# ma-compbio/MATCHA

Hardware: AMD Instinct MI355X
Metric: training hyperedges/sec at k∈{2..5}, embed_dim=64; 1/2/4/8 MI355X (higher is better)
Workload: dtype f32; 1 GPU; hg38_1mb bins (N=3067), k in {2,3,4,5} mixed-k zero-padded to L=5, embed_dim=64, front end=table, neg_num=3, dropout on, AdamW lr=1e-3, 400000 known hyperedges; parallelism=dp1, hipgraph=False, table_gradient_exchange=none, embedding_backward=float atomics, exchange_overlapped=False

## Files before the change

matcha_amd/csrc/tail_bwd.hip:

```cpp
#include "bf16x3.hpp"
#include "kernels.hpp"
#include "loss_reduce.hpp"

namespace matcha {

namespace {

constexpr int kLd = 68;
constexpr int kTileF = 32 * kLd;
constexpr int kPS = 80;
constexpr int kPlane = 32 * kPS;
constexpr int kPT = 3 * kPlane;
constexpr float kEps = 1e-5f;
constexpr int kSlab = 2 * 4096 + 10 * 64;
constexpr int kVec = 2 * 4096;
typedef Planes<kPS, 16> PL;

struct TailBwdArgs {
  const float* dH2; const float* Y; const float* H1;
  const int32_t* count; const int32_t* half_meta; const int32_t* tok_slot;
  int nhalves;
  const float* W0; const float* W1;
  const uint64_t* seed; float p_fc1, p_pff;
  float* ddyn0; float* slab;
  float* zero_rows;
  int64_t zero_floats;
  const float* row_loss; int64_t B; float* losses; int zero_recon;
  const float* vslab;
};
constexpr size_t kLdsBytes = (size_t)2 * kTileF * 4 + (size_t)4 * kPT * 2;

__global__ __launch_bounds__(256) __attribute__((amdgpu_waves_per_eu(2, 2))) void tail_bwd64_kernel(TailBwdArgs g) {
  extern __shared__ __attribute__((aligned(16))) float lds[];
  float* Hs = lds;
  float* Ds = lds + kTileF;
  short* Dp = reinterpret_cast<short*>(lds + 2 * kTileF);
  short* Hp = Dp + kPT;
  short* Yp = Hp + kPT;
  short* Zp = Yp + kPT;

  const int tid = threadIdx.x;
  const int nwg = (int)gridDim.x - (g.losses ? 1 : 0);
  if ((int)blockIdx.x == nwg) {
    loss_reduce_role<256>(g.row_loss, g.B, g.losses, g.zero_recon, lds);
    return;
  }
  const int tr = g.count[1];
  int nh = g.count[3];
  if (nh > g.nhalves) nh = g.nhalves;
  const int per = (nh + nwg - 1) / nwg;
  const int tile_lo = blockIdx.x * per;
  const int tile_hi = tile_lo + per < nh ? tile_lo + per : nh;

  if (g.zero_floats > 0) {
    f32x4* z = reinterpret_cast<f32x4*>(g.zero_rows);
    const int64_t n4 = g.zero_floats >> 2;
    for (int64_t i = (int64_t)blockIdx.x * 256 + tid; i < n4; i += (int64_t)nwg * 256) z[i] = (f32x4){0.f, 0.f, 0.f, 0.f};
  }
  const bool zero_tok = g.zero_rows && g.zero_floats == 0;
  if (blockIdx.x == 0 && tid < 16)
    *reinterpret_cast<f32x4*>(g.ddyn0 + (int64_t)tr * 64 + 4 * tid) = (f32x4){0.f, 0.f, 0.f, 0.f};
  const bool drop1 = g.p_fc1 > 0.f, drop2 = g.p_pff > 0.f;
  uint32_t key1 = 0, key2 = 0, thr1 = 0, thr2 = 0;
  float ks1 = 1.f, ks2 = 1.f;
  if (drop1 || drop2) {
    const uint64_t seed = *g.seed;
    key1 = rng_key(seed, kStreamDropFc1); key2 = rng_key(seed, kStreamDropPff);
    if (drop1) { thr1 = dropout_threshold(g.p_fc1); ks1 = 1.f / (1.f - g.p_fc1); }
    if (drop2) { thr2 = dropout_threshold(g.p_pff); ks2 = 1.f / (1.f - g.p_pff); }
  }
  const float unscale = drop2 ? 1.f - g.p_pff : 1.f;

  f32x4 aw1[4], aw0[4];
#pragma unroll
  for (int i = 0; i < 4; ++i) { aw1[i] = (f32x4){0.f, 0.f, 0.f, 0.f}; aw0[i] = aw1[i]; }
  float va0 = 0.f, va1 = 0.f, va2 = 0.f;
  V8 a_c1 = zero8();
  f32x4 a_c0 = {0.f, 0.f, 0.f, 0.f};

  Frag3 W1f[2], W0f[2];
  {
    const int lane = tid & 63, wave = tid >> 6, c16 = lane & 15, kq = lane >> 4, fb = 16 * wave;
    const float* p1 = g.W1 + (8 * kq) * 64 + fb + c16;
    const float* p0 = g.W0 + (8 * kq) * 64 + fb + c16;
#pragma unroll
    for (int s = 0; s < 2; ++s) {
      float v1[8], v0[8];
#pragma unroll
      for (int j = 0; j < 8; ++j) { v1[j] = p1[(32 * s + j) * 64]; v0[j] = p0[(32 * s + j) * 64]; }
      W1f[s] = split8(v1); W0f[s] = split8(v0);
    }
  }

  const int4* meta = reinterpret_cast<const int4*>(g.half_meta);
  const int4 mzero = make_int4(0, 0, 0, 0);
  int4 mc = tile_lo < tile_hi ? meta[tile_lo] : mzero;
  int4 mn = tile_lo + 1 < tile_hi ? meta[tile_lo + 1] : mzero;
  V8 yn, hn, dn;
  uint32_t sn0 = 0, sn1 = 0;
#define TB_GLOAD(M)                                                                                      \
  do {                                                                                                   \
    const int row__ = tid >> 3, sub__ = tid & 7;                                                         \
    const int64_t tok__ = (M).x + (row__ < (M).y ? row__ : ((M).y > 0 ? (M).y - 1 : 0));                  \
    const int64_t o__ = tok__ * 64 + 8 * sub__;                                                          \
    yn = ld8(g.Y + o__); hn = ld8(g.H1 + o__); dn = ld8(g.dH2 + o__);                                    \
    if (drop1 || drop2) {      \
      const int c16__ = tid & 15;                                                                        \
      sn0 = (uint32_t)g.tok_slot[(M).x + (c16__ < (M).y ? c16__ : 0)];                                   \
      sn1 = (uint32_t)g.tok_slot[(M).x + (16 + c16__ < (M).y ? 16 + c16__ : 0)];                         \
    }                                                                                                    \
  } while (0)
  TB_GLOAD(mc);
  V8 yq = yn, hq = hn, dq = dn;
  uint32_t sq0 = sn0, sq1 = sn1;
  {
    const V8 ty = yn, th = hn, td = dn; const uint32_t t0_ = sn0, t1_ = sn1;
    TB_GLOAD(mn);
    yq = yn; hq = hn; dq = dn; sq0 = sn0; sq1 = sn1;
    yn = ty; hn = th; dn = td; sn0 = t0_; sn1 = t1_;
  }

  for (int tile = tile_lo; tile < tile_hi; ++tile) {
    const int4 mnn = tile + 2 < tile_hi ? meta[tile + 2] : mzero;
    const int t0 = mc.x, n_real = mc.y;
    const float* vs = g.vslab + (int64_t)tile * kSlab + kVec;
    const float vl0 = vs[tid], vl1 = vs[tid + 256], vl2 = tid == 64 ? vs[9 * 64] : 0.f;
    int tid_ = tid;
    asm volatile("" : "+v"(tid_));
    const int lane = tid_ & 63, wave = tid_ >> 6;
    const int c16 = lane & 15, kq = lane >> 4, fb = 16 * wave;
    const int row = tid_ >> 3, sub = tid_ & 7;
    {
      const V8 dh2 = scale8(row < n_real ? 1.f : 0.f, dn);
      if (zero_tok && row < n_real) st8(g.zero_rows + ((int64_t)t0 + row) * 64 + 8 * sub, zero8());
      add8(a_c1, dh2);
      st8(&Ds[row * kLd + 8 * sub], dh2);
      st8(&Hs[row * kLd + 8 * sub], hn);
      PL::store(Dp + row * kPS + 8 * sub, split8(dh2));
      PL::store(Hp + row * kPS + 8 * sub, split8(hn));
      PL::store(Yp + row * kPS + 8 * sub, split8(yn));
    }
    const uint32_t slot0 = sn0, slot1 = sn1;
    __syncthreads();
    yn = yq; hn = hq; dn = dq; sn0 = sq0; sn1 = sq1;
    {
      const V8 ty = yn, th = hn, td = dn; const uint32_t t0_ = sn0, t1_ = sn1;
      TB_GLOAD(mnn);
      yq = yn; hq = hn; dq = dn; sq0 = sn0; sq1 = sn1;
      yn = ty; hn = th; dn = td; sn0 = t0_; sn1 = t1_;
    }
    {
      f32x4 acc0 = {0.f, 0.f, 0.f, 0.f}, acc1 = acc0;
      const short* dp = Dp + c16 * kPS + 8 * kq;
#pragma unroll
      for (int s = 0; s < 2; ++s) {
        const Frag3 b0 = PL::row(dp + 32 * s), b1 = PL::row(dp + 16 * kPS + 32 * s);
        acc0 = mma6(acc0, W1f[s], b0); acc1 = mma6(acc1, W1f[s], b1);
      }
      const f32x4 hv0 = *reinterpret_cast<const f32x4*>(&Hs[c16 * kLd + fb + 4 * kq]);
      const f32x4 hv1 = *reinterpret_cast<const f32x4*>(&Hs[(16 + c16) * kLd + fb + 4 * kq]);
      const uint32_t hr0 = lowbias32(slot0 ^ key2), hr1 = lowbias32(slot1 ^ key2);
#pragma unroll
      for (int e = 0; e < 4; ++e) {
        const uint32_t f = (uint32_t)(fb + 4 * kq + e);
        float v0 = acc0[e], v1 = acc1[e];
        if (drop2) {
          v0 = lowbias32(f ^ hr0) >= thr2 ? v0 * ks2 : 0.f;
          v1 = lowbias32(f ^ hr1) >= thr2 ? v1 * ks2 : 0.f;
        }
        const float t0_ = hv0[e] * unscale, t1_ = hv1[e] * unscale;
        acc0[e] = v0 * (1.f - t0_ * t0_); acc1[e] = v1 * (1.f - t1_ * t1_);
      }
      a_c0 += acc0 + acc1;
      {
        const P3 p0 = split2(acc0[0], acc0[1]), p1 = split2(acc0[2], acc0[3]);
        short* d = Zp + c16 * kPS + fb + 4 * kq;
        *reinterpret_cast<u32x2*>(d) = (u32x2){p0.h, p1.h}; *reinterpret_cast<u32x2*>(d + kPlane) = (u32x2){p0.m, p1.m};
        *reinterpret_cast<u32x2*>(d + 2 * kPlane) = (u32x2){p0.l, p1.l};
      }
      {
        const P3 p0 = split2(acc1[0], acc1[1]), p1 = split2(acc1[2], acc1[3]);
        short* d = Zp + (16 + c16) * kPS + fb + 4 * kq;
        *reinterpret_cast<u32x2*>(d) = (u32x2){p0.h, p1.h}; *reinterpret_cast<u32x2*>(d + kPlane) = (u32x2){p0.m, p1.m};
        *reinterpret_cast<u32x2*>(d + 2 * kPlane) = (u32x2){p0.l, p1.l};
      }
    }
    __syncthreads();
    {
      f32x4 acc0 = *reinterpret_cast<const f32x4*>(&Ds[c16 * kLd + fb + 4 * kq]);
      f32x4 acc1 = *reinterpret_cast<const f32x4*>(&Ds[(16 + c16) * kLd + fb + 4 * kq]);
      const short* zp = Zp + c16 * kPS + 8 * kq;
#pragma unroll
      for (int s = 0; s < 2; ++s) {
        const Frag3 b0 = PL::row(zp + 32 * s), b1 = PL::row(zp + 16 * kPS + 32 * s);
        acc0 = mma6(acc0, W0f[s], b0); acc1 = mma6(acc1, W0f[s], b1);
      }
      if (drop1) {
        const uint32_t hr0 = lowbias32(slot0 ^ key1), hr1 = lowbias32(slot1 ^ key1);
#pragma unroll
        for (int e = 0; e < 4; ++e) {
          const uint32_t f = (uint32_t)(fb + 4 * kq + e);
          acc0[e] = lowbias32(f ^ hr0) >= thr1 ? acc0[e] * ks1 : 0.f;
          acc1[e] = lowbias32(f ^ hr1) >= thr1 ? acc1[e] * ks1 : 0.f;
        }
      }
      float* out = g.ddyn0 + ((int64_t)t0 + c16) * 64 + fb + 4 * kq;
      if (c16 < n_real) *reinterpret_cast<f32x4*>(out) = acc0;
      if (16 + c16 < n_real) *reinterpret_cast<f32x4*>(out + 16 * 64) = acc1;
    }
    {
      const int blk = ((4 * kq + ((lane & 15) >> 2)) * kPS) + 4 * (lane & 3);
      const Frag3 hb = PL::col(Hp + blk + fb), yb = PL::col(Yp + blk + fb);
#pragma unroll
      for (int i = 0; i < 4; ++i) aw1[i] = mma6(aw1[i], PL::col(Dp + blk + 16 * i), hb);
#pragma unroll
      for (int i = 0; i < 4; ++i) aw0[i] = mma6(aw0[i], PL::col(Zp + blk + 16 * i), yb);
    }
    __syncthreads();
    va0 += vl0; va1 += vl1; va2 += vl2;
    mc = mn; mn = mnn;
  }
#undef TB_GLOAD

  const int lane = tid & 63, wave = tid >> 6, c16 = lane & 15, kq = lane >> 4, fb = 16 * wave;
  float* slab = g.slab + (int64_t)blockIdx.x * kSlab;
  {
    const int col = fb + c16;
#pragma unroll
    for (int i = 0; i < 4; ++i)
#pragma unroll
      for (int reg = 0; reg < 4; ++reg) {
        const int rw = 16 * i + 4 * kq + reg;
        slab[rw * 64 + col] = aw1[i][reg];
        slab[4096 + rw * 64 + col] = aw0[i][reg];
      }
  }
  float* red = lds;
  {
    const int sub = tid & 7;
    const float t[8] = {a_c1.a.x, a_c1.a.y, a_c1.b.x, a_c1.b.y, a_c1.c.x, a_c1.c.y, a_c1.d.x, a_c1.d.y};
#pragma unroll
    for (int e = 0; e < 8; ++e) {
      float x = t[e];
      x += __shfl_xor(x, 8, 64); x += __shfl_xor(x, 16, 64); x += __shfl_xor(x, 32, 64);
      if (lane < 8) red[wave * 64 + 8 * sub + e] = x;
    }
  }
  {
#pragma unroll
    for (int e = 0; e < 4; ++e) {
      float x = a_c0[e];
      x += __shfl_xor(x, 1, 64); x += __shfl_xor(x, 2, 64); x += __shfl_xor(x, 4, 64); x += __shfl_xor(x, 8, 64);
      if (c16 == 0) slab[kVec + 8 * 64 + fb + 4 * kq + e] = x;
    }
  }
  {
    slab[kVec + tid] = va0;
    if (tid < 192) slab[kVec + 256 + tid] = va1;
    if (tid == 64) slab[kVec + 9 * 64] = va2;
  }
  __syncthreads();
  if (tid < 64) slab[kVec + 7 * 64 + tid] = (red[tid] + red[64 + tid]) + (red[128 + tid] + red[192 + tid]);
}

}

int tail_bwd_grid() { return 2 * device_cu_count(); }
size_t tail_bwd_slab_floats() { return (size_t)tail_bwd_grid() * kSlab; }

int launch_tail_bwd64(const matcha_tensors& p, const float* dH2, const float* Y, const float* H1, const Ragged& rg, const uint64_t* seed, float p_fc1,
                      float p_pff, float* ddyn0, float* slab, const float* vslab, float* zero_rows, int64_t zero_floats, hipStream_t st, const float* row_loss, int64_t B,
                      float* losses, bool zero_recon) {
  TailBwdArgs g;
  g.row_loss = row_loss; g.B = B; g.losses = losses; g.zero_recon = zero_recon ? 1 : 0;
  g.vslab = vslab; g.zero_rows = zero_rows; g.zero_floats = zero_rows ? zero_floats : 0;
  MATCHA_CHECK_ARG(zero_floats >= 0 && zero_floats % 4 == 0, "tail backward: the zeroed range is a whole number of float4");
  g.dH2 = dH2; g.Y = Y; g.H1 = H1; g.count = rg.count; g.half_meta = rg.half_meta; g.tok_slot = rg.tok_slot; g.nhalves = rg.nhalves;
  g.W0 = p.pff0_w; g.W1 = p.pff1_w; g.seed = seed; g.p_fc1 = p_fc1; g.p_pff = p_pff;
  g.ddyn0 = ddyn0; g.slab = slab;
  ProfScope ps(MATCHA_PROF_FUSED_FWD, 0.0, st);
  auto kfn = tail_bwd64_kernel;
  (void)hipFuncSetAttribute(reinterpret_cast<const void*>(kfn), hipFuncAttributeMaxDynamicSharedMemorySize, 160 * 1024);
  hipLaunchKernelGGL(kfn, dim3(tail_bwd_grid() + (losses ? 1 : 0)), dim3(256), kLdsBytes, st, g);
  MATCHA_CHECK_LAUNCH("tail_bwd64_kernel");
  return MATCHA_OK;
}

}
```

Measured before the change: 62.39 million hyperedges/s.

## Restructure tail backward loop into ping-pong register stages with buffer-descriptor stores

Rewrites the per-tile loop of the tail backward kernel as a two-way unrolled walk with two register row buffers (A/B). The next tile's staging into LDS now follows a barrier at the end of each trip, which removes the separate end-of-loop barrier and the register shuffling of prefetched rows. It also reads metadata with readfirstlane so it is wave-uniform, prefetches meta three tiles ahead, always loads token slots, specialises the loop on zero_tok at compile time, and writes d_dyn through raw buffer stores that use an out-of-range offset instead of branches. It adds optional timing instrumentation and a host check that the buffer size stays under 2^31 bytes, at the cost of larger code and more register pressure.

```diff
diff --git a/matcha_amd/csrc/tail_bwd.hip b/matcha_amd/csrc/tail_bwd.hip
--- a/matcha_amd/csrc/tail_bwd.hip
+++ b/matcha_amd/csrc/tail_bwd.hip
@@ -1,6 +1,7 @@
 #include "bf16x3.hpp"
 #include "kernels.hpp"
 #include "loss_reduce.hpp"
+#include <type_traits>
 
 namespace matcha {
 
@@ -15,11 +16,20 @@
 constexpr int kSlab = 2 * 4096 + 10 * 64;
 constexpr int kVec = 2 * 4096;
 typedef Planes<kPS, 16> PL;
+constexpr int kRsrcRaw32 = 0x00020000;
+constexpr uint32_t kOffPastAny = 0x80000000u;
+
+#ifdef TB_TIMING
+#define TB_T(i) do { const long long now__ = wall_clock64(); tph[i] += now__ - tlast; tlast = now__; } while (0)
+#else
+#define TB_T(i) do { } while (0)
+#endif
 
 struct TailBwdArgs {
   const float* dH2; const float* Y; const float* H1;
   const int32_t* count; const int32_t* half_meta; const int32_t* tok_slot;
   int nhalves;
+  int tok_cap;
   const float* W0; const float* W1;
   const uint64_t* seed; float p_fc1, p_pff;
   float* ddyn0; float* slab;
@@ -92,63 +102,63 @@
     }
   }
 
-  const int4* meta = reinterpret_cast<const int4*>(g.half_meta);
-  const int4 mzero = make_int4(0, 0, 0, 0);
-  int4 mc = tile_lo < tile_hi ? meta[tile_lo] : mzero;
-  int4 mn = tile_lo + 1 < tile_hi ? meta[tile_lo + 1] : mzero;
-  V8 yn, hn, dn;
-  uint32_t sn0 = 0, sn1 = 0;
-#define TB_GLOAD(M)                                                                                      \
+#ifdef TB_TIMING
+  long long tph[7] = {0, 0, 0, 0, 0, 0, 0};
+  long long tlast = wall_clock64();
+#endif
+  const int tr_rows = tr < g.tok_cap ? tr : g.tok_cap;
+  const __amdgpu_buffer_rsrc_t dyn_rsrc = __builtin_amdgcn_make_buffer_rsrc(g.ddyn0, 0, (tr_rows + 1) * 256, kRsrcRaw32);
+  struct Rows { V8 y, h, d; uint32_t s0, s1; };
+  auto meta_raw = [&](int i) __attribute__((always_inline)) {
+    return *reinterpret_cast<const int2*>(g.half_meta + 4 * (int64_t)(i < tile_hi ? i : tile_hi));
+  };
+  auto meta_of = [&](const int2 raw, int i) __attribute__((always_inline)) {
+    const int x = __builtin_amdgcn_readfirstlane(raw.x), y = __builtin_amdgcn_readfirstlane(raw.y);
+    return make_int2(i < tile_hi ? x : 0, i < tile_hi ? y : 0);
+  };
+#define TB_GLOAD(R, M)                                                                                   \
   do {                                                                                                   \
-    const int row__ = tid >> 3, sub__ = tid & 7;                                                         \
+    const int row__ = tid >> 3, sub__ = tid & 7, c16__ = tid & 15;                                       \
+    (R).s0 = (uint32_t)g.tok_slot[(M).x + (c16__ < (M).y ? c16__ : 0)];                                  \
+    (R).s1 = (uint32_t)g.tok_slot[(M).x + (16 + c16__ < (M).y ? 16 + c16__ : 0)];                        \
     const int64_t tok__ = (M).x + (row__ < (M).y ? row__ : ((M).y > 0 ? (M).y - 1 : 0));                  \
     const int64_t o__ = tok__ * 64 + 8 * sub__;                                                          \
-    yn = ld8(g.Y + o__); hn = ld8(g.H1 + o__); dn = ld8(g.dH2 + o__);                                    \
-    if (drop1 || drop2) {      \
-      const int c16__ = tid & 15;                                                                        \
-      sn0 = (uint32_t)g.tok_slot[(M).x + (c16__ < (M).y ? c16__ : 0)];                                   \
-      sn1 = (uint32_t)g.tok_slot[(M).x + (16 + c16__ < (M).y ? 16 + c16__ : 0)];                         \
+    (R).y = ld8(g.Y + o__); (R).h = ld8(g.H1 + o__); (R).d = ld8(g.dH2 + o__);                           \
+  } while (0)
+#define TB_STAGE(R, M, ZT)                                                                               \
+  do {                                                                                                   \
+    int tis__ = tid;                                                                                     \
+    asm volatile("" : "+v"(tis__));                                                                      \
+    const int row__ = tis__ >> 3, sub__ = tis__ & 7;                                                     \
+    const V8 dh2__ = scale8(row__ < (M).y ? 1.f : 0.f, (R).d);                                           \
+    if ((ZT) && row__ < (M).y) {                                                                         \
+      float z__ = 0.f;                                                                                   \
+      asm volatile("" : "+v"(z__));       \
+      V8 zz__; zz__.a = f2{z__, z__}; zz__.b = zz__.a; zz__.c = zz__.a; zz__.d = zz__.a;                 \
+      st8(g.zero_rows + ((int64_t)(M).x + row__) * 64 + 8 * sub__, zz__);                                \
     }                                                                                                    \
+    add8(a_c1, dh2__);                                                                                   \
+    st8(&Ds[row__ * kLd + 8 * sub__], dh2__);                                                            \
+    st8(&Hs[row__ * kLd + 8 * sub__], (R).h);                                                            \
+    PL::store(Dp + row__ * kPS + 8 * sub__, split8(dh2__));                                              \
+    PL::store(Hp + row__ * kPS + 8 * sub__, split8((R).h));                                              \
+    PL::store(Yp + row__ * kPS + 8 * sub__, split8((R).y));                                              \
   } while (0)
-  TB_GLOAD(mc);
-  V8 yq = yn, hq = hn, dq = dn;
-  uint32_t sq0 = sn0, sq1 = sn1;
-  {
-    const V8 ty = yn, th = hn, td = dn; const uint32_t t0_ = sn0, t1_ = sn1;
-    TB_GLOAD(mn);
-    yq = yn; hq = hn; dq = dn; sq0 = sn0; sq1 = sn1;
-    yn = ty; hn = th; dn = td; sn0 = t0_; sn1 = t1_;
-  }
-
-  for (int tile = tile_lo; tile < tile_hi; ++tile) {
-    const int4 mnn = tile + 2 < tile_hi ? meta[tile + 2] : mzero;
+
+  auto trip = [&](int tile, const int2 mc, const int2 mnn, int2& raw3, Rows& S) __attribute__((always_inline)) {
     const int t0 = mc.x, n_real = mc.y;
-    const float* vs = g.vslab + (int64_t)tile * kSlab + kVec;
-    const float vl0 = vs[tid], vl1 = vs[tid + 256], vl2 = tid == 64 ? vs[9 * 64] : 0.f;
+    TB_T(0);
+    __syncthreads();
+    TB_T(1);
+    const uint32_t slot0 = S.s0, slot1 = S.s1;
     int tid_ = tid;
     asm volatile("" : "+v"(tid_));
     const int lane = tid_ & 63, wave = tid_ >> 6;
     const int c16 = lane & 15, kq = lane >> 4, fb = 16 * wave;
-    const int row = tid_ >> 3, sub = tid_ & 7;
-    {
-      const V8 dh2 = scale8(row < n_real ? 1.f : 0.f, dn);
-      if (zero_tok && row < n_real) st8(g.zero_rows + ((int64_t)t0 + row) * 64 + 8 * sub, zero8());
-      add8(a_c1, dh2);
-      st8(&Ds[row * kLd + 8 * sub], dh2);
-      st8(&Hs[row * kLd + 8 * sub], hn);
-      PL::store(Dp + row * kPS + 8 * sub, split8(dh2));
-      PL::store(Hp + row * kPS + 8 * sub, split8(hn));
-      PL::store(Yp + row * kPS + 8 * sub, split8(yn));
-    }
-    const uint32_t slot0 = sn0, slot1 = sn1;
-    __syncthreads();
-    yn = yq; hn = hq; dn = dq; sn0 = sq0; sn1 = sq1;
-    {
-      const V8 ty = yn, th = hn, td = dn; const uint32_t t0_ = sn0, t1_ = sn1;
-      TB_GLOAD(mnn);
-      yq = yn; hq = hn; dq = dn; sq0 = sn0; sq1 = sn1;
-      yn = ty; hn = th; dn = td; sn0 = t0_; sn1 = t1_;
-    }
+    const float* vs = g.vslab + (int64_t)tile * kSlab + kVec;
+    const float vl0 = vs[tid_], vl1 = vs[tid_ + 256], vl2r = vs[tid_ == 64 ? 9 * 64 : tid_];
+    raw3 = meta_raw(tile + 3);
+    TB_GLOAD(S, mnn);
     {
       f32x4 acc0 = {0.f, 0.f, 0.f, 0.f}, acc1 = acc0;
       const short* dp = Dp + c16 * kPS + 8 * kq;
@@ -185,7 +195,9 @@
         *reinterpret_cast<u32x2*>(d + 2 * kPlane) = (u32x2){p0.l, p1.l};
       }
     }
+    TB_T(2);
     __syncthreads();
+    TB_T(3);
     {
       f32x4 acc0 = *reinterpret_cast<const f32x4*>(&Ds[c16 * kLd + fb + 4 * kq]);
       f32x4 acc1 = *reinterpret_cast<const f32x4*>(&Ds[(16 + c16) * kLd + fb + 4 * kq]);
@@ -204,10 +216,11 @@
           acc1[e] = lowbias32(f ^ hr1) >= thr1 ? acc1[e] * ks1 : 0.f;
         }
       }
-      float* out = g.ddyn0 + ((int64_t)t0 + c16) * 64 + fb + 4 * kq;
-      if (c16 < n_real) *reinterpret_cast<f32x4*>(out) = acc0;
-      if (16 + c16 < n_real) *reinterpret_cast<f32x4*>(out + 16 * 64) = acc1;
-    }
+      const uint32_t off = ((uint32_t)t0 + (uint32_t)c16) * 256u + 4u * (uint32_t)(fb + 4 * kq);
+      __builtin_amdgcn_raw_buffer_store_b128(__builtin_bit_cast(u32x4, acc0), dyn_rsrc, c16 < n_real ? off : kOffPastAny, 0, 0);
+      __builtin_amdgcn_raw_buffer_store_b128(__builtin_bit_cast(u32x4, acc1), dyn_rsrc, 16 + c16 < n_real ? off + 16u * 256u : kOffPastAny, 0, 0);
+    }
+    TB_T(4);
     {
       const int blk = ((4 * kq + ((lane & 15) >> 2)) * kPS) + 4 * (lane & 3);
       const Frag3 hb = PL::col(Hp + blk + fb), yb = PL::col(Yp + blk + fb);
@@ -216,11 +229,56 @@
 #pragma unroll
       for (int i = 0; i < 4; ++i) aw0[i] = mma6(aw0[i], PL::col(Zp + blk + 16 * i), yb);
     }
-    __syncthreads();
-    va0 += vl0; va1 += vl1; va2 += vl2;
-    mc = mn; mn = mnn;
+    va0 += vl0; va1 += vl1; va2 += tid_ == 64 ? vl2r : 0.f;
+    TB_T(5);
+  };
+
+  auto walk = [&](auto zt_c) __attribute__((always_inline)) {
+    constexpr bool ZT = decltype(zt_c)::value;
+    int tile = tile_lo;
+    int2 ra = meta_raw(tile), rb = meta_raw(tile + 1);
+    int2 mc = meta_of(ra, tile), mn = meta_of(rb, tile + 1);
+    Rows A, B;
+    TB_GLOAD(A, mc);
+    ra = meta_raw(tile + 2);
+    TB_GLOAD(B, mn);
+    TB_STAGE(A, mc, ZT);
+    int2 mnn;
+    while (tile + 2 < tile_hi) {
+      mnn = meta_of(ra, tile + 2);
+      trip(tile, mc, mnn, rb, A);
+      __syncthreads();
+      TB_T(1);
+      TB_STAGE(B, mn, ZT);
+      mc = mn; mn = mnn;
+      mnn = meta_of(rb, tile + 3);
+      trip(tile + 1, mc, mnn, ra, B);
+      __syncthreads();
+      TB_T(1);
+      TB_STAGE(A, mn, ZT);
+      mc = mn; mn = mnn;
+      tile += 2;
+    }
+    mnn = meta_of(ra, tile + 2);
+    trip(tile, mc, mnn, rb, A);
+    if (tile + 1 < tile_hi) {
+      __syncthreads();
+      TB_T(1);
+      TB_STAGE(B, mn, ZT);
+      trip(tile + 1, mn, mnn, ra, B);
+    }
+  };
+  if (tile_lo < tile_hi) {
+    if (zero_tok) walk(std::true_type{}); else walk(std::false_type{});
   }
 #undef TB_GLOAD
+#undef TB_STAGE
+  __syncthreads();
+#ifdef TB_TIMING
+  if (blockIdx.x == 0 && (tid == 0 || tid == 192))
+    printf("tail_bwd64 wg0 wave %d us: stage %.1f barrier-wait %.1f loads+dZ1 %.1f d-dyn %.1f weight-grads %.1f (halves %d)\n", tid >> 6, tph[0] * 0.01,
+           (tph[1] + tph[3]) * 0.01, tph[2] * 0.01, tph[4] * 0.01, tph[5] * 0.01, tile_hi - tile_lo);
+#endif
 
   const int lane = tid & 63, wave = tid >> 6, c16 = lane & 15, kq = lane >> 4, fb = 16 * wave;
   float* slab = g.slab + (int64_t)blockIdx.x * kSlab;
@@ -278,6 +336,9 @@
   g.dH2 = dH2; g.Y = Y; g.H1 = H1; g.count = rg.count; g.half_meta = rg.half_meta; g.tok_slot = rg.tok_slot; g.nhalves = rg.nhalves;
   g.W0 = p.pff0_w; g.W1 = p.pff1_w; g.seed = seed; g.p_fc1 = p_fc1; g.p_pff = p_pff;
   g.ddyn0 = ddyn0; g.slab = slab;
+  MATCHA_CHECK_ARG(rg.nhalves >= 0 && ((int64_t)31 * rg.nhalves + 1) * 256 < (int64_t)kOffPastAny,
+                   "tail backward: d dyn is addressed through a buffer descriptor of < 2^31 bytes");
+  g.tok_cap = 31 * rg.nhalves;
   ProfScope ps(MATCHA_PROF_FUSED_FWD, 0.0, st);
   auto kfn = tail_bwd64_kernel;
   (void)hipFuncSetAttribute(reinterpret_cast<const void*>(kfn), hipFuncAttributeMaxDynamicSharedMemorySize, 160 * 1024);
```

Result: no change. 62.62 million hyperedges/s (median of 6 runs) (+0.4%).
